# johnviljoen/f16_mpc_oop_py

Hardware: AMD Instinct MI355X
Metric: F16 env steps/sec (hifi Nguyen model, explicit Euler dt=1ms, batch 4096 per GPU) (higher is better)
Workload: dtype f64

## Files before the change

f16_mpc_oop_py_amd/csrc/f16_dynamics.hip:

```cpp
#include <hip/hip_runtime.h>
#include <stdlib.h>

#include <type_traits>

#include "../../include/f16_hip.h"
#include "f16_ctx.h"
#include "f16_plant.hpp"
#include "f16_rollout_common.hpp"
#include "f16_plant_quad.hpp"
#include "f16_mppi.hpp"
#include "f16_gain_sched.hpp"

namespace f16 {

struct CostArgs : SchedArgs {
  const double *x0;
  const double *x_ref;
  const double *u_ref;
  double *x_end;
  long B0, ld0;
  f16_cost_weights w;
};
struct GainSchedArgs : SchedArgs {
  f16_gain_grid grid;
// ... 533 lines not shown
#pragma unroll
        for (int k = 0; k < 3; ++k) { ls[k] = xt[k][lane]; ldm[k] = xt[3 + k][lane]; ts[k] = xt[6 + k][lane]; td[k] = xt[9 + k][lane]; }
        Totals tt;
        compose_totals(ls, ldm, ts, td, a.xcg, tt);
        if (wave == 0) {
          if (live) {
            p.qbar = xt[12][lane]; p.ps = xt[13][lane];
            st |= xst[0][lane] | xst[1][lane] | xst[2][lane] | xst[3][lane];
            plant_forces(xa, p, tt.Cx, tt.Cy, tt.Cz, xd);
#pragma unroll
            for (int k = 0; k < 9; ++k) x[k] += xd[k] * a.dt;
          }
        } else {
          if (live) {
            plant_moments(x[9], x[10], x[11], xt[12][lane], tt.Cl, tt.Cm, tt.Cn, xd);
#pragma unroll
            for (int k = 9; k < 12; ++k) x[k] += xd[k] * a.dt;
          }
          if (tr && --until_store == 0) {
            until_store = a.traj_every;
            if (valid) {
#pragma unroll
              for (int k = 9; k < 12; ++k) __builtin_nontemporal_store(x[k], tr + k * a.ld);
            }
            tr += 18 * a.ld;
          }
        }
      }
    }
#ifdef F16_EXP_STAMP4W
    if (lane == 0 && blockIdx.x == 0 && a.traj) {
      double *d = a.traj + 18 * a.ld * 2 + wave * 4;
      d[0] = (double)tD; d[1] = (double)tA; d[2] = (double)tB; d[3] = (double)tC;
    }
#endif
    if (valid && wave != 1) {
      bool finite = true;
      const int k0 = wave == 0 ? 0 : (wave == 2 ? 9 : 12), k1 = wave == 0 ? 9 : (wave == 2 ? 12 : 18);
#pragma unroll
      for (int k = 0; k < 18; ++k)
        if (k >= k0 && k < k1) { finite = finite && isfinite(x[k]); a.out[k * a.ld + b] = x[k]; }
      if (st & ST_ENVELOPE) st |= envelope_state_bits(x) & (((1 << k1) - (1 << k0)) << 8);
      if (a.status) atomicOr(&a.status[b], st | (finite ? 0 : ST_NONFINITE));
      if (LQR && wave == 3 && a.u_out) {
        a.u_out[b] = u[0];
#pragma unroll
        for (int i = 0; i < 3; ++i) a.u_out[(1 + i) * a.ld + b] = ul[i];
      }
    }
    __syncthreads();
  }
}

template <int GROUPS, bool LQR = false, bool SCHED = false>
__global__ __launch_bounds__(256 * GROUPS) void k_rollout_q(RolloutArgs<SCHED> a) {
  constexpr int NA = 16 * GROUPS;
  constexpr bool G1 = GROUPS == 1;
  __shared__ __attribute__((aligned(16))) double tab[TABLE_IMAGE_DOUBLES];
  __shared__ double xs[18][NA], xt[11][NA];
  __shared__ int xenv[3][NA], xst[2][NA];
  __shared__ double xpsi[G1 ? 4 : 3][NA];
#ifdef F16_EXP_STAMPQ
  const unsigned long long tstage0 = __builtin_amdgcn_s_memtime();
#endif
  {
    const double2 *src = reinterpret_cast<const double2 *>(a.tab);
    double2 *dst = reinterpret_cast<double2 *>(tab);
    for (int i = threadIdx.x; i < TABLE_IMAGE_DOUBLES / 2; i += 256 * GROUPS) dst[i] = src[i];
    __syncthreads();
  }
#ifdef F16_EXP_STAMPQ
  const unsigned long long tstage = __builtin_amdgcn_s_memtime() - tstage0;
#endif
  const int role = G1 ? __builtin_amdgcn_readfirstlane((threadIdx.x >> 6) & 3) : (threadIdx.x >> 6) & 3;
  const int grp = threadIdx.x >> 8, lane = threadIdx.x & 63, ac = 16 * grp + (lane >> 2), s = lane & 3;
  const bool envchk = !(a.flags & FLAG_NO_ENVELOPE);
  for (long b0 = (long)blockIdx.x * NA; b0 < a.B; b0 += (long)gridDim.x * NA) {
    const bool valid = b0 + ac < a.B;
    const long b = valid ? b0 + ac : a.B - 1;
    double x[18];
#pragma unroll
    for (int k = 0; k < 18; ++k) x[k] = a.out[k * a.ld + b];
    double ucmd = a.u[s * a.ld + b];
    double kr0 = 0, kr1 = 0, kr2 = 0, dm0 = 0, dm1 = 0, dm2 = 0, ulast = ucmd;
    if (LQR && role == 3) {
      const long row = 9 * (s > 0 ? s - 1 : 0) + 4;
      kr0 = a.K[row * a.ld + b]; kr1 = a.K[(row + 1) * a.ld + b]; kr2 = a.K[(row + 2) * a.ld + b];
      dm0 = a.dem[b]; dm1 = a.dem[a.ld + b]; dm2 = a.dem[2 * a.ld + b];
    }
    double xact = s == 0 ? x[12] : (s == 1 ? x[13] : (s == 2 ? x[14] : x[15]));
    int st = a.status ? a.status[b] : 0;
    double *tr = a.traj ? a.traj + b : nullptr;
    int until_store = a.traj_every;
    QuadCell qc = quad_cell_none();
    LongCorners klong = {};
    LatCorners klat = {};
    RowAhead<1, false> ra;
    double dmq = 0;
    const int rs = LQR && s == 3 ? 2 : s;
    if constexpr (SCHED) {
      dmq = s == 0 ? dm0 : (s == 1 ? dm1 : dm2);
      ra.init(a, LQR ? 3 : 4, a.out + b, rs * a.ld, role == 3);
      ra.settle();
    }
#ifdef F16_EXP_STAMPQ
    unsigned long long tA = 0, tB = 0, tC = 0, tD = 0, t0 = __builtin_amdgcn_s_memtime();
#if F16_EXP_STAMPQ + 0 == 2
#define QSTAMP_WAIT 0xC07F
#else
#define QSTAMP_WAIT 0
#endif
#define QSTAMP(acc) { __builtin_amdgcn_s_waitcnt(QSTAMP_WAIT); unsigned long long t1 = __builtin_amdgcn_s_memtime(); acc += t1 - t0; t0 = t1; }
#else
#define QSTAMP(acc)
#endif
    if constexpr (G1) {
      switch (role) {
        case 0: {
          constexpr int wave = 0;
#include "f16_quad_steps.inc"
        } break;
        case 1: {
          constexpr int wave = 1;
#include "f16_quad_steps.inc"
        } break;
        case 2: {
          constexpr int wave = 2;
#include "f16_quad_steps.inc"
        } break;
        default: {
          constexpr int wave = 3;
#include "f16_quad_steps.inc"
        } break;
      }
    } else {
      const int wave = role;
#include "f16_quad_steps.inc"
    }
#ifdef F16_EXP_STAMPQ
    if (lane == 0 && blockIdx.x == 0 && a.traj) {
      double *d = a.traj + 18 * a.ld * 2 + role * 4;
      d[0] = (double)tD; d[1] = (double)tA; d[2] = (double)tB; d[3] = (double)tC;
      a.traj[18 * a.ld * 2 + a.ld + role] = (double)tstage;
    }
#endif
    if (valid) {
      if (role == 2 && s == 0) {
        bool finite = true;
#pragma unroll
        for (int k = 0; k < 9; ++k) { finite = finite && isfinite(x[k]); a.out[k * a.ld + b] = x[k]; }
        if (st & ST_ENVELOPE) st |= envelope_state_bits(x) & (0x1FF << 8);
        if (a.status) atomicOr(&a.status[b], st | (finite ? 0 : ST_NONFINITE));
      } else if (role == 1 && s == 0) {
        bool finite = true;
#pragma unroll
        for (int k = 9; k < 12; ++k) { finite = finite && isfinite(x[k]); a.out[k * a.ld + b] = x[k]; }
        if (st & ST_ENVELOPE) st |= envelope_state_bits(x) & (0x7 << 17);
        if (a.status) atomicOr(&a.status[b], st | (finite ? 0 : ST_NONFINITE));
      } else if (role == 3) {
        a.out[(12 + s) * a.ld + b] = xact;
        bool finite = isfinite(xact);
        if (s < 2) { const double v = s == 0 ? x[16] : x[17]; finite = finite && isfinite(v); a.out[(16 + s) * a.ld + b] = v; }
        if (st & ST_ENVELOPE) {
          const double lim = s == 1 ? 25.0 : (s == 2 ? 21.5 : 30.0);
          if (s == 0 ? (xact < 1000 || xact > 19000) : (xact < -lim || xact > lim)) st |= 1 << (8 + 12 + s);
          if (s == 0 && (x[16] < 0. || x[16] > 25)) st |= 1 << (8 + 16);
        }
        if (a.status) atomicOr(&a.status[b], st | (finite ? 0 : ST_NONFINITE));
        if (LQR && a.u_out) a.u_out[s * a.ld + b] = ulast;
      }
    }
    __syncthreads();
  }
}

struct LinArgsL {
  double *x;
  const double *Ad, *Bd, *K, *xref, *u0;
  double *trx, *tru;
  long B, ld;
  int nsteps, every;
  unsigned track;
};
__global__ __launch_bounds__(64, 1) void k_rollout_lqr_linear(LinArgsL a) {
  const long b = (long)blockIdx.x * 64 + threadIdx.x;
  if (b >= a.B) return;
  double A[81], Bm[27], K[27], x[9], xr[9], u0[3];
#pragma unroll
  for (int e = 0; e < 81; ++e) A[e] = a.Ad[e * a.ld + b];
#pragma unroll
  for (int e = 0; e < 27; ++e) { Bm[e] = a.Bd[e * a.ld + b]; K[e] = a.K[e * a.ld + b]; }
#pragma unroll
  for (int j = 0; j < 9; ++j) { x[j] = a.x[j * a.ld + b]; xr[j] = a.xref[j * a.ld + b]; }
#pragma unroll
// ... 70 lines not shown
  if (int rc = check_common(ctx, x, xdot, B, ld)) return rc;
  if (!u) return set_error(F16_EINVAL, "u is NULL");
  if (B == 0) return F16_OK;
  DynArgs a = base_args<DynArgs>(ctx, B, ld, xcg, fi_flag, flags, status);
  a.x = x; a.u = u; a.out = xdot;
  const Geometry g = geometry(B, fi_flag);
  by_block(g, [&](auto block) {
    constexpr int BLOCK = decltype(block)::value;
    if (fi_flag == 0) hipLaunchKernelGGL((k_xdot<BLOCK, 0>), dim3(g.grid), dim3(BLOCK), 0, (hipStream_t)stream, a);
    else hipLaunchKernelGGL((k_xdot<BLOCK, -1>), dim3(g.grid), dim3(BLOCK), 0, (hipStream_t)stream, a);
  });
  return hip_check(hipGetLastError(), "f16_xdot_batch launch");
}

extern "C" int f16_nlplant_batch(f16_ctx *ctx, const double *xu, double *xdot, int32_t *status, long B, long ld,
                                 double xcg, int fi_flag, unsigned flags, void *stream) {
  if (int rc = check_common(ctx, xu, xdot, B, ld)) return rc;
  if (B == 0) return F16_OK;
  DynArgs a = base_args<DynArgs>(ctx, B, ld, xcg, fi_flag, flags, status);
  a.x = xu; a.out = xdot;
  if (B <= 256) {
    hipLaunchKernelGGL((k_nlplant<64, false>), dim3((unsigned)((B + 63) / 64)), dim3(64), 0, (hipStream_t)stream, a);
  } else {
    const Geometry g = geometry(B, fi_flag);
    by_block(g, [&](auto block) {
      constexpr int BLOCK = decltype(block)::value;
      hipLaunchKernelGGL((k_nlplant<BLOCK, true>), dim3(g.grid), dim3(BLOCK), 0, (hipStream_t)stream, a);
    });
  }
  return hip_check(hipGetLastError(), "f16_nlplant_batch launch");
}

#ifdef F16_RK4_512
constexpr bool RK4_512 = true;
#else
constexpr bool RK4_512 = false;
#endif
template <bool LQR, bool SCHED, bool COST, int STAGES = 1, bool GS = false>
static int rollout_dispatch(f16_ctx *ctx, RolloutArgsGS<SCHED, COST, GS> &a, void *stream) {
  const hipStream_t st = (hipStream_t)stream;
  const long B = a.B;
  const bool hifi = a.fi == 1;
  static const long max4w = [] { const char *e = getenv("F16_ROLLOUT_4W_MAXB"); return e ? atol(e) : 64L * 256; }();
  static const long maxq = [] { const char *e = getenv("F16_ROLLOUT_QUAD_MAXB"); return e ? atol(e) : 16L * 256; }();
  const char *const what = COST ? "f16_rollout_cost launch" : "f16_rollout launch";
  if (a.flags & F16_FLAG_ONE_LANE) {
    if constexpr (GS) hipLaunchKernelGGL((k_rollout_exact_gs<STAGES>), one_lane_grid(B), dim3(64), 0, st, a);
    else
    hipLaunchKernelGGL((k_rollout_exact<LQR, SCHED, COST, STAGES>), one_lane_grid(B), dim3(64), 0, st, a);
    return hip_check(hipGetLastError(), what);
  }
  if constexpr (!COST && STAGES == 1 && !GS) {
    if (hifi && B <= 2 * maxq) {
      if (B <= maxq) hipLaunchKernelGGL((k_rollout_q<1, LQR, SCHED>), dim3((unsigned)((B + 15) / 16)), dim3(256), 0, st, a);
      else hipLaunchKernelGGL((k_rollout_q<2, LQR, SCHED>), dim3((unsigned)((B + 31) / 32)), dim3(512), 0, st, a);
      return hip_check(hipGetLastError(), what);
    }
    if (hifi && B <= max4w) {
      hipLaunchKernelGGL((k_rollout_4w<LQR, SCHED>), dim3((unsigned)((B + 63) / 64)), dim3(256), 0, st, a);
      return hip_check(hipGetLastError(), what);
    }
  }
  constexpr bool WIDE = STAGES == 1 || RK4_512;
  Geometry g = geometry(B, a.fi, WIDE ? 512 : 256);
#ifdef F16_FAST_DIV
  static const int use_i32 = [] { const char *e = getenv("F16_ROLLOUT_I32"); return e ? atoi(e) : 1; }();
  if constexpr (WIDE) if (hifi && use_i32 && g.block == 512) {
    a.tab32 = ctx->d_tab32;
    if constexpr (GS) hipLaunchKernelGGL((k_rollout_i_gs<512, STAGES>), dim3(g.grid), dim3(512), 0, st, a);
    else
    hipLaunchKernelGGL((k_rollout_i<512, LQR, SCHED, COST, STAGES>), dim3(g.grid), dim3(512), 0, st, a);
    return hip_check(hipGetLastError(), what);
  }
#endif
  if (LQR && g.block == 512) g.block = 256;
  by_block(g, [&](auto block) {
    constexpr int BLOCK = decltype(block)::value;
    if constexpr (GS && BLOCK < 512) {
      if (a.fi == 0) hipLaunchKernelGGL((k_rollout_gs<BLOCK, 0, STAGES>), dim3(g.grid), dim3(BLOCK), 0, st, a);
      else hipLaunchKernelGGL((k_rollout_gs<BLOCK, -1, STAGES>), dim3(g.grid), dim3(BLOCK), 0, st, a);
    } else
    if constexpr (!((LQR || !WIDE) && BLOCK == 512)) {
      if (a.fi == 0) hipLaunchKernelGGL((k_rollout<BLOCK, 0, LQR, SCHED, COST, STAGES>), dim3(g.grid), dim3(BLOCK), 0, st, a);
      else hipLaunchKernelGGL((k_rollout<BLOCK, -1, LQR, SCHED, COST, STAGES>), dim3(g.grid), dim3(BLOCK), 0, st, a);
    }
  });
  return hip_check(hipGetLastError(), what);
}

struct PlantRollout {
  const char *missing;
  const double *x;
  const double *u;
  double *out;
  double *traj;
  int32_t *status;
  long B, ld;
  int nsteps, traj_every;
  double dt, xcg;
  int fi;
  unsigned flags;
  const double *seq = nullptr;
  int hold = 1;
  const double *K = nullptr, *dem = nullptr;
  double *u_out = nullptr;
  long B0 = 0, ld0 = 0;
  const double *x_ref = nullptr, *u_ref = nullptr;
// ... 217 lines not shown
```

f16_mpc_oop_py_amd/csrc/f16_plant.hpp:

```cpp
#pragma once
#include <hip/hip_runtime.h>

#include "f16_tables.h"

namespace f16 {

constexpr int ST_ALPHA1 = 1, ST_ALPHA2 = 2, ST_BETA = 4, ST_EL = 8, ST_ENVELOPE = 16, ST_NONFINITE = 32;
constexpr unsigned FLAG_FIX_CLR = 1u, FLAG_NO_ENVELOPE = 2u, FLAG_NO_CELL_CACHE = 16u;

#define F16_DEV __device__ __forceinline__

#ifdef F16_FAST_DIV
#define F16_DIVC(x, c) ((x) * (1.0 / (c)))
#else
#define F16_DIVC(x, c) ((x) / (c))
#endif

__device__ __forceinline__ double f16_rcp(double x) {
#ifdef F16_FAST_DIV
  double r = __builtin_amdgcn_rcp(x);
  r = fma(r, fma(-x, r, 1.0), r);
  r = fma(r, fma(-x, r, 1.0), r);
  return r;
#else
// ... 29 lines not shown
  static F16_DEV double kvv(double k, double b, double c) { return fma_svv(k, b, c); }
};
struct KVector {
  static F16_DEV double vvk(double a, double b, double k) { return fma_vvv(a, b, k); }
  static F16_DEV double kvv(double k, double b, double c) { return fma_vvv(k, b, c); }
};
F16_DEV void in_vgpr(double &x) { asm volatile("" : "+v"(x)); }
template <typename T>
F16_DEV void table_in_vgprs(T &t) {
  double *d = reinterpret_cast<double *>(&t);
#pragma unroll
  for (unsigned i = 0; i < sizeof(T) / sizeof(double); ++i) in_vgpr(d[i]);
}

struct PowK {
  double log2e, ln2_hi, ln2_lo, nln2_hi, nln2_lo, two_thirds;
  double E[10];
  double L[7];
};
constexpr PowK POW_K = {
    1.44269504088896338700e+00, 6.93147180559945286227e-01, 2.31904681384629955842e-17, -6.93147180559945286227e-01,
    -2.31904681384629955842e-17, 6.66666666666666629659e-01,
    {2.50223225676461415e-08, 2.76309034901126543e-07, 2.75575145458253105e-06, 2.48014910390950412e-05, 1.98412695891155217e-04,
     1.38888889459163820e-03, 8.33333333345504315e-03, 4.16666666665197541e-02, 1.66666666666664770e-01, 5.00000000000001221e-01},
    {1.53670161652585818e-01, 1.52503063567000663e-01, 1.81863527724766383e-01, 2.22221384831011309e-01, 2.85714293974435540e-01,
     3.99999999961319630e-01, 6.66666666666728247e-01}};

struct LogQuot {
  double h, l;
  int e;
};
template <typename OP = KScalar>
F16_DEV LogQuot log_k_quot(const PowK &K, double x) {
  const double m = __builtin_amdgcn_frexp_mant(x);
  const bool lo = m < K.two_thirds;
  const double sc = lo ? 2.0 : 1.0;
  const int e = __builtin_amdgcn_frexp_exp(x) + (lo ? -1 : 0);
  const double ym1 = fma(m, sc, -1.0), yp1 = fma(m, sc, 1.0);
  const double ylo = fma(m, sc, -(yp1 + -1.0));
  double r = __builtin_amdgcn_rcp(yp1);
  r = fma(fma(-yp1, r, 1.0), r, r);
  r = fma(fma(-yp1, r, 1.0), r, r);
  const double q = ym1 * r;
  const double p = yp1 * q;
  const double pl = fma(q, ylo, fma(q, yp1, -p));
  const double s25 = fma(yp1, q, pl);
  const double s27 = pl - fma(-yp1, q, s25);
  const double d28 = ym1 - s25;
  const double d32 = d28 + (((ym1 - d28) - s25) - s27);
  const double h = fma(r, d32, q);
  const double l = fma(r, d32, -fma(-ym1, r, h));
  return {h, l, e};
}
template <typename OP = KScalar>
F16_DEV double log_k_sum(const PowK &K, double x, const LogQuot &qt) {
  const double h = qt.h, l = qt.l;
  const int e = qt.e;
  const double z = h * h;
  double c = OP::vvk(z, K.L[0], K.L[1]);
#pragma unroll
  for (int k = 2; k < 7; ++k) c = OP::vvk(z, c, K.L[k]);
  const double a44 = __builtin_ldexp(h, 1), a45 = __builtin_ldexp(l, 1);
  const double t46 = h * z;
  const double u48 = fma(t46, c, a44);
  const double u50 = fma(t46, c, -(u48 - a44));
  const double u51 = a45 + u50;
  const double u52 = u48 + u51;
  const double u54 = u51 - (u52 - u48);
  const double f = (double)e;
  const double g56n = f * K.nln2_hi;
  const double g59 = OP::kvv(K.ln2_lo, f, OP::kvv(K.ln2_hi, f, g56n));
  const double g60 = OP::kvv(K.ln2_hi, f, g59);
  const double g62 = g59 - OP::kvv(K.nln2_hi, f, g60);
  const double w63 = g60 + u52;
  const double w64 = w63 - g60;
  const double w68 = (u52 - w64) + (g60 - (w63 - w64));
  const double v69 = g62 + u54;
  const double v70 = v69 - g62;
  const double v74 = (u54 - v70) + (g62 - (v69 - v70));
  const double k75 = v69 + w68;
  const double k76 = w63 + k75;
  const double k80 = k76 + (v74 + (k75 - (k76 - w63)));
  double res = __builtin_fabs(x) == __builtin_inf() ? x : k80;
  res = x < 0.0 ? __builtin_nan("") : res;
  return x == 0.0 ? -__builtin_inf() : res;
}
template <typename OP = KScalar>
F16_DEV double log_k(const PowK &K, double x) {
  return log_k_sum<OP>(K, x, log_k_quot<OP>(K, x));
}

template <typename OP = KScalar>
F16_DEV double exp_k(const PowK &K, double x) {
  const double n = rint(x * K.log2e);
  const double r = OP::kvv(K.nln2_lo, n, OP::kvv(K.nln2_hi, n, x));
  double c = OP::vvk(r, K.E[0], K.E[1]);
#pragma unroll
  for (int k = 2; k < 10; ++k) c = OP::vvk(r, c, K.E[k]);
  c = fma(r, c, 1.0);
  c = fma(r, c, 1.0);
  double res = __builtin_ldexp(c, (int)n);
  res = x > 1024.0 ? __builtin_inf() : res;
  return x < -1075.0 ? 0.0 : res;
}

struct AtmosAlt {
  double tfac, temp, t4;
};
F16_DEV AtmosAlt atmos_alt(double alt) {
  AtmosAlt h;
  h.tfac = 1 - .703e-5 * alt;
  h.temp = 519.0 * h.tfac;
  if (alt >= 35000.0) h.temp = 390;
#ifdef F16_FAST_POW
// ... 897 lines not shown
```

f16_mpc_oop_py_amd/csrc/f16_plant_quad.hpp:

```cpp
#pragma once
#include "f16_plant.hpp"

namespace f16 {

template <int J>
F16_DEV double quad_bcast(double v) {
  constexpr int ctrl = J | (J << 2) | (J << 4) | (J << 6);
  int lo = __double2loint(v), hi = __double2hiint(v);
  lo = __builtin_amdgcn_mov_dpp(lo, ctrl, 0xF, 0xF, true);
  hi = __builtin_amdgcn_mov_dpp(hi, ctrl, 0xF, 0xF, true);
  return __hiloint2double(hi, lo);
}

template <int J>
F16_DEV int quad_bcast_i(int v) {
  constexpr int ctrl = J | (J << 2) | (J << 4) | (J << 6);
  return __builtin_amdgcn_mov_dpp(v, ctrl, 0xF, 0xF, true);
}

F16_DEV void quad_taken_here_1(double &v) { asm volatile("" : "+v"(v)); }
F16_DEV void quad_taken_here_1(int &v) { asm volatile("" : "+v"(v)); }
template <typename... T>
F16_DEV void quad_taken_here(T &...v) { (quad_taken_here_1(v), ...); }

F16_DEV void quad_store_sample(const double (&smp)[5], double *tr, int s, long ld) {
#pragma unroll
  for (int j = 0; j < 5; ++j) {
    const int kk = s + 4 * j;
    if (kk < 18) __builtin_nontemporal_store(smp[j], tr + kk * ld);
  }
}

struct QuadBr { BrCell c; int ja, jb, jd; bool offa, offb, offd; };
template <bool USE_D2, typename TP>
F16_DEV BrRaw quad_br_load(TP T, double alpha, double beta, double el, int s, int &nX, double &vX) {
  const int ax = s < 2 ? s : 2;
  const int gel = USE_D2 ? (int)(el >= 0.0) : (el >= -10.0) + (el >= 0.0) + (el >= 10.0);
  const int offX = ax == 0 ? OFF_BP_A1 : (ax == 1 ? OFF_BP_B1 : (USE_D2 ? OFF_BP_D2 : OFF_BP_D1));
  nX = ax == 0 ? N_A1 : (ax == 1 ? N_B1 : (USE_D2 ? N_D2 : N_D1));
  vX = ax == 0 ? alpha : (ax == 1 ? beta : el);
  const int gX = ax == 0 ? alpha_guess(alpha) : (ax == 1 ? beta_guess(beta) : gel);
  return br_load(T + offX, nX, gX);
}
F16_DEV QuadBr quad_br_cells(const BrRaw &r, int nX, double vX) {
  QuadBr q;
  bool off;
  q.c = br_cell(r, nX, vX, off);
  q.ja = quad_bcast_i<0>(q.c.j); q.jb = quad_bcast_i<1>(q.c.j); q.jd = quad_bcast_i<2>(q.c.j);
  const int o = off ? 1 : 0;
  q.offa = quad_bcast_i<0>(o) != 0; q.offb = quad_bcast_i<1>(o) != 0; q.offd = quad_bcast_i<2>(o) != 0;
  return q;
}

struct QuadCell { int ja, jb, jd; double x0, x1; };
F16_DEV QuadCell quad_cell_none() { QuadCell c; c.ja = c.jb = c.jd = 0; c.x0 = c.x1 = __builtin_nan(""); return c; }
template <bool USE_D2, bool CACHE, typename TP>
F16_DEV QuadBr quad_br_cached(TP T, double alpha, double beta, double el, int s, unsigned flags, QuadCell &cc, bool &hit) {
  const double v = s == 0 ? alpha : (s == 1 ? beta : el);
  const bool in = cc.x0 <= v && v < cc.x1;
  QuadBr q;
  hit = CACHE && !(flags & FLAG_NO_CELL_CACHE) && __builtin_amdgcn_ballot_w64(!in) == 0;
  if (hit) {
    q.c.j = 0; q.c.v = v; q.c.x0 = cc.x0; q.c.x1 = cc.x1;
    q.ja = cc.ja; q.jb = cc.jb; q.jd = cc.jd;
    q.offa = q.offb = q.offd = false;
  } else {
    int nX; double vX;
    const BrRaw rx = quad_br_load<USE_D2>(T, alpha, beta, el, s, nX, vX);
    F16_PHASE();
    q = quad_br_cells(rx, nX, vX);
    if (CACHE) { cc.ja = q.ja; cc.jb = q.jb; cc.jd = q.jd; cc.x0 = q.c.x0; cc.x1 = q.c.x1; }
  }
  return q;
}
F16_DEV void quad_br_axes(const QuadBr &q, Axis &a, Axis &b, Axis &d) {
  const Axis own = br_axis(q.c);
  a.j = q.ja; a.l = quad_bcast<0>(own.l); a.m = quad_bcast<0>(own.m);
  b.j = q.jb; b.l = quad_bcast<1>(own.l); b.m = quad_bcast<1>(own.m);
  d.j = q.jd; d.l = quad_bcast<2>(own.l); d.m = quad_bcast<2>(own.m);
}

struct LongCorners {
  Q4 qlo, qhi, q0, qlef;
  double g0, g1, m0, m1, h0, h1, e0, e1, r0, r1, p0, p1, b0, b1, hr0, hr1, hp0, hp1, a45;
};
struct LatCorners {
  Q4 qlo, qhi, q0, qy, qr, qa, ql, qal;
  double a45;
};

template <bool PIN>
F16_DEV double lerp_d(double f1, double f2, const Axis &a) {
  if constexpr (PIN) return __builtin_fma(a.l, f2, a.m * f1);
  else return lerp(f1, f2, a);
}

struct QuadIn {
  double alpha, beta, el, dail, drud, dlef, P, Q, R, kq, kb;
};
F16_DEV QuadIn quad_inputs(const double *xu) {
  const double B = 30.0, cbar = 11.32, r2d = 180.0 / 3.141592653589793;
  QuadIn in;
  double vt = xu[6];
  if (vt <= 0.01) vt = 0.01;
  in.alpha = xu[7] * r2d; in.beta = xu[8] * r2d;
  in.P = xu[9]; in.Q = xu[10]; in.R = xu[11];
  in.el = xu[13];
  in.dail = F16_DIVC(xu[14], 21.5);
  in.drud = F16_DIVC(xu[15], 30.0);
  in.dlef = 1 - F16_DIVC(xu[16], 25.0);
#ifdef F16_FAST_DIV
  const double r2vt = f16_rcp(2 * vt);
  in.kq = cbar * r2vt; in.kb = B * r2vt;
#else
  in.kq = cbar / (2 * vt); in.kb = B / (2 * vt);
#endif
  return in;
}

#ifdef F16_EXP_STAMPQ2
__device__ unsigned long long g_qstamp[8];
#define Q2STAMP(i) { __builtin_amdgcn_s_waitcnt(0); const unsigned long long t1_ = __builtin_amdgcn_s_memtime(); if (blockIdx.x == 0 && (threadIdx.x & 63) == 0) g_qstamp[i] += t1_ - tq_; tq_ = t1_; }
#else
#define Q2STAMP(i)
#endif
template <bool CACHE, typename TP>
F16_DEV double quad_long(TP T, const double *xu, int s, double xcg, unsigned flags, QuadCell &cc, LongCorners &kept, double &latd,
                         int &status) {
#ifdef F16_EXP_STAMPQ2
  unsigned long long tq_ = __builtin_amdgcn_s_memtime();
#endif
  const QuadIn in = quad_inputs(xu);
  Q2STAMP(0)
  const int k = s < 2 ? s : 2;
  bool hit;
  const QuadBr qb = quad_br_cached<false, CACHE>(T, in.alpha, in.beta, in.el, s, flags, cc, hit);
  Q2STAMP(1)
  LongCorners fresh;
  LongCorners &c = CACHE ? kept : fresh;
  const bool hi_a = qb.ja > N_A2 - 2;
  if (!CACHE || !hit) {
    c.a45 = T[OFF_BP_A1 + N_A2 - 1];
    const int j2 = hi_a ? N_A2 - 2 : qb.ja;
    const int n1 = qb.jb * N_A1 + qb.ja, n2 = qb.jb * N_A2 + j2;
    struct { int j; } ca = {qb.ja}, cd = {qb.jd};
    constexpr int SA = S_G3A, SB = S_G3A * N_A1, SD = S_G3A * N_A1 * N_B1;
    TP p = T + OFF_G3A + n1 * SA + k;
    c.qlo = ld4(p + cd.j * SD, SA, SB); c.qhi = ld4(p + (cd.j + 1) * SD, SA, SB); c.q0 = ld4(p + D1_ZERO_NODE * SD, SA, SB);
    c.qlef = ld4(T + OFF_G2B + n2 * S_G2B + k, S_G2B, S_G2B * N_A2);
    TP g = T + OFF_G1A + ca.j * S_G1A, h = T + OFF_G1B + j2 * S_G1B;
    c.g0 = g[3 * k]; c.g1 = g[S_G1A + 3 * k]; c.m0 = g[11]; c.m1 = g[S_G1A + 11];
    c.h0 = h[3 * k]; c.h1 = h[S_G1B + 3 * k];
    c.e0 = T[OFF_ETA + cd.j]; c.e1 = T[OFF_ETA + cd.j + 1];
    const int ir = k == 0 ? 1 : (k == 1 ? 7 : 4), ib = k == 1 ? 9 : 10;
    c.r0 = g[ir]; c.r1 = g[S_G1A + ir]; c.p0 = g[ir + 1]; c.p1 = g[S_G1A + ir + 1]; c.b0 = g[ib]; c.b1 = g[S_G1A + ib];
    c.hr0 = h[ir]; c.hr1 = h[S_G1B + ir]; c.hp0 = h[ir + 1]; c.hp1 = h[S_G1B + ir + 1];
  }
  if (qb.offa) status |= ST_ALPHA1 | ST_ALPHA2;
  if (qb.offb) status |= ST_BETA;
  if (qb.offd) status |= ST_EL;
  if (hi_a && in.alpha > c.a45) status |= ST_ALPHA2;
  Q2STAMP(2)
  F16_PHASE();
  Axis a1, b, d1;
  quad_br_axes(qb, a1, b, d1);
  Axis a2 = a1;
  if (hi_a) { a2.j = N_A2 - 2; a2.l = 1.0; a2.m = 0.0; }
  const W4 W1 = bil_weights(a1, b), W2 = bil_weights(a2, b);
  const double Cf = lerp_d<CACHE>(bil4w(c.qlo, a1, b, W1), bil4w(c.qhi, a1, b, W1), d1);
  const double C0 = bil4w(c.q0, a1, b, W1);
  const double dC = bil4w(c.qlef, a2, b, W2) - C0;
  const double Cq = lerp(c.g0, c.g1, a1), dCm = lerp(c.m0, c.m1, a1), dq = lerp(c.h0, c.h1, a2), eta = lerp(c.e0, c.e1, d1);
  const double dql = k == 1 ? dC : dq;
  double tot = Cf * (k == 2 ? eta : 1.0) + dC * in.dlef + in.kq * (Cq + dql * in.dlef) * in.Q + (k == 2 ? dCm : 0.0);
  const double Cz_tot = quad_bcast<1>(tot);
  if (k == 2) tot += Cz_tot * (0.35 - xcg);
  double Cr = lerp(c.r0, c.r1, a1);
  if (k == 2 && !(flags & FLAG_FIX_CLR)) Cr = 0.0;
  const double Cp = lerp(c.p0, c.p1, a1), Cb = lerp(c.b0, c.b1, a1);
  const double dCr = lerp(c.hr0, c.hr1, a2), dCp = lerp(c.hp0, c.hp1, a2);
  latd = in.kb * (Cr + dCr * in.dlef) * in.R + in.kb * (Cp + dCp * in.dlef) * in.P + (k == 0 ? 0.0 : Cb * in.beta);
  Q2STAMP(3)
  return tot;
}

template <bool CACHE, typename TP>
F16_DEV double quad_lat(TP T, const double *xu, int s, unsigned flags, QuadCell &cc, LatCorners &kept, int &status) {
  const QuadIn in = quad_inputs(xu);
  const int k = s < 2 ? s : 2;
  bool hit;
  const QuadBr qb = quad_br_cached<true, CACHE>(T, in.alpha, in.beta, in.el, s, flags, cc, hit);
  LatCorners fresh;
  LatCorners &c = CACHE ? kept : fresh;
  const bool hi_a = qb.ja > N_A2 - 2;
  if (!CACHE || !hit) {
    c.a45 = T[OFF_BP_A1 + N_A2 - 1];
    const int j2 = hi_a ? N_A2 - 2 : qb.ja;
    const int n1 = qb.jb * N_A1 + qb.ja, n2 = qb.jb * N_A2 + j2;
    struct { int j; } cd = {qb.jd};
    constexpr int SA3 = S_G3B, SB3 = S_G3B * N_A1, SD3 = S_G3B * N_A1 * N_B1;
    TP p3 = T + OFF_G3B + n1 * SA3 + (k > 0 ? k - 1 : 0);
    c.qlo = ld4(p3 + cd.j * SD3, SA3, SB3); c.qhi = ld4(p3 + (cd.j + 1) * SD3, SA3, SB3); c.q0 = ld4(p3 + D2_ZERO_NODE * SD3, SA3, SB3);
    constexpr int SA2 = S_G2A, SB2 = S_G2A * N_A1;
    TP pa = T + OFF_G2A + n1 * SA2;
    c.qy = ld4(pa, SA2, SB2); c.qr = ld4(pa + 1 + k, SA2, SB2); c.qa = ld4(pa + 4 + k, SA2, SB2);
    constexpr int SAB = S_G2B, SBB = S_G2B * N_A2;
    TP pb = T + OFF_G2B + n2 * SAB;
    c.ql = ld4(pb + 3 + k, SAB, SBB); c.qal = ld4(pb + 6 + k, SAB, SBB);
  }
  if (qb.offa) status |= ST_ALPHA1 | ST_ALPHA2;
  if (qb.offb) status |= ST_BETA;
  if (qb.offd) status |= ST_EL;
  if (hi_a && in.alpha > c.a45) status |= ST_ALPHA2;
  F16_PHASE();
  Axis a1, b, d2;
  quad_br_axes(qb, a1, b, d2);
  Axis a2 = a1;
  if (hi_a) { a2.j = N_A2 - 2; a2.l = 1.0; a2.m = 0.0; }
  const W4 W1 = bil_weights(a1, b), W2 = bil_weights(a2, b);
  const double C3 = lerp_d<CACHE>(bil4w(c.qlo, a1, b, W1), bil4w(c.qhi, a1, b, W1), d2), C30 = bil4w(c.q0, a1, b, W1);
  const double Cy = bil4w(c.qy, a1, b, W1), Cr30 = bil4w(c.qr, a1, b, W1), Ca20 = bil4w(c.qa, a1, b, W1);
  const double Clef = bil4w(c.ql, a2, b, W2), Ca20lef = bil4w(c.qal, a2, b, W2);
  const double base = k == 0 ? Cy : C3, base0 = k == 0 ? Cy : C30;
  const double dlefC = Clef - base0;
  const double dr30 = Cr30 - base0;
  const double da20 = Ca20 - base0, da20lef = Ca20lef - Clef - da20;
  return base + dlefC * in.dlef + (da20 + da20lef * in.dlef) * in.dail + dr30 * in.drud;
}

}
```

f16_mpc_oop_py_amd/csrc/f16_quad_steps.inc:

```
    [[maybe_unused]] SinCosK ksc = {};
    [[maybe_unused]] PowK kpw = {};
    [[maybe_unused]] bool env_h = false;
    [[maybe_unused]] AtmosAlt ah = {};
    [[maybe_unused]] LogQuot lq = {};
    if constexpr (G1) {
      if (wave == 0 || wave == 2) ksc = reloaded(QUAD_K.sc);
      if (wave == 3) kpw = reloaded(QUAD_K.pw);
      if (wave == 2) table_in_vgprs(ksc);
      if (wave == 0) { in_vgpr(ksc.S[7]); in_vgpr(ksc.C[8]); }
      if (wave == 3) { in_vgpr(kpw.E[0]); in_vgpr(kpw.L[0]); }
      if (wave == 0 && s == 0) {
        double sp, cp;
        F16_SINCOS_K(ksc, x[5], &sp, &cp);
        xpsi[1][ac] = sp; xpsi[2][ac] = cp;
      }
      if (wave == 2) {
        env_h = envchk && (x[2] < 0 || x[2] > 100000);
        if (s == 0) {
#pragma unroll
          for (int k = 0; k < 6; ++k) xs[k][ac] = x[k];
        }
      }
      if (wave == 3) {
        ah = atmos_alt(x[2]);
        lq = log_k_quot(kpw, ah.tfac);
        quad_taken_here(ah.tfac, ah.temp, ah.t4, lq.h, lq.l, lq.e);
      }
      if (wave != 3) {
#pragma unroll
        for (int k = 0; k < 18; ++k)
          if (!(wave == 2 ? k < 9 : (wave == 1 && k >= 9 && k < 12))) x[k] = 0;
      }
    }
    for (int t = 0; t <= a.nsteps; ++t) {
      if (wave == 2) {
        if constexpr (G1) {
          xenv[0][ac] = env_h | (envchk & ((x[6] < 0) | (x[6] > 900) | (x[7] < -20.) | (x[7] > 90) | (x[8] < -30.) | (x[8] > 30)));
          xs[6 + (s < 3 ? s : 2)][ac] = s == 0 ? x[6] : (s == 1 ? x[7] : x[8]);
        } else {
          xenv[0][ac] = envchk && (x[2] < 0 || x[2] > 100000 || x[6] < 0 || x[6] > 900 || x[7] < -20. || x[7] > 90 ||
                                   x[8] < -30. || x[8] > 30);
          if (s == 0) {
#pragma unroll
            for (int k = 0; k < 9; ++k) xs[k][ac] = x[k];
          }
        }
      } else if (wave == 1) {
        xenv[1][ac] = envchk && (x[9] < -300 || x[9] > 300 || x[10] < -100 || x[10] > 100 || x[11] < -50 || x[11] > 50);
        if (s < 3) xs[9 + s][ac] = s == 0 ? x[9] : (s == 1 ? x[10] : x[11]);
      } else if (wave == 3) {
        const double lim = s == 1 ? 25.0 : (s == 2 ? 21.5 : 30.0);
        const bool bad = s == 0 ? (xact < 1000 || xact > 19000) : (xact < -lim || xact > lim);
        const bool badl = x[16] < 0. || x[16] > 25;
        if (s == 0) xenv[2][ac] = 0;
        xs[12 + s][ac] = xact;
        if (s < 2) xs[16 + s][ac] = s == 0 ? x[16] : x[17];
        __builtin_amdgcn_wave_barrier();
        if (envchk && (bad || badl)) xenv[2][ac] = 1;
      }
      QSTAMP(tD)
      __syncthreads();
      QSTAMP(tA)
      double xa[17];
      int env_any = 0;
      if constexpr (G1) {
        env_any = xenv[0][ac] | xenv[1][ac] | xenv[2][ac];
#pragma unroll
        for (int k = 0; k < 17; ++k) xa[k] = xs[k][ac];
        if (wave == 2) { xa[3] = x[3]; xa[4] = x[4]; xa[6] = x[6]; xa[7] = x[7]; xa[8] = x[8]; }
        if (wave == 1) { xa[9] = x[9]; xa[10] = x[10]; xa[11] = x[11]; }
      }
      [[maybe_unused]] double smp[5] = {0, 0, 0, 0, 0};
      [[maybe_unused]] bool sample_due = false;
      if constexpr (G1) {
        if (wave == 2) {
#pragma unroll
          for (int j = 0; j < 5; ++j) smp[j] = xs[s + 4 * j < 18 ? s + 4 * j : s][ac];
          asm volatile("" ::: "memory");
        }
      }
      if (wave == 2 && tr && t > 0 && --until_store == 0) {
        until_store = a.traj_every;
        if constexpr (G1) {
          sample_due = true;
        } else {
          if (valid) {
#pragma unroll
            for (int j = 0; j < 5; ++j) {
              const int kk = s + 4 * j;
              if (kk < 18) __builtin_nontemporal_store(xs[kk][ac], tr + kk * a.ld);
            }
          }
          tr += 18 * a.ld;
        }
      }
      if (t == a.nsteps) {
        if constexpr (G1) {
          if (sample_due && valid) quad_store_sample(smp, tr, s, a.ld);
        }
        break;
      }
      if constexpr (!G1) {
        env_any = xenv[0][ac] | xenv[1][ac] | xenv[2][ac];
#pragma unroll
        for (int k = 0; k < 17; ++k) xa[k] = xs[k][ac];
      }
      if ((!G1 || wave != 0) && env_any) st |= ST_ENVELOPE;
      const bool live = !(st & ST_ENVELOPE);
      double xd[9] = {0, 0, 0, 0, 0, 0, 0, 0, 0};
      double U = 0, V = 0, W = 0, s_t = 0, c_t = 0, s_phi = 0, c_phi = 0, cb = 0, vtc = 0, r1 = 0, r2 = 0, r3 = 0;
      double fu0 = 0, fv0 = 0, fw0 = 0, mo0 = 0, mo1 = 0, mo2 = 0;
      bool newrow = false;
      if constexpr (SCHED) newrow = ra.due(a, LQR ? 3 : 4);
      if (wave == 0) {
        int sa_ = 0;
        double latd;
        const double tot = quad_long<G1>((const double *)tab, xa, s, a.xcg, a.flags, qc, klong, latd, sa_);
        if (s < 3) { xt[s][ac] = tot; xt[8 + s][ac] = latd; }
        xst[0][ac] = sa_;
      } else if (wave == 1) {
        int sa_ = 0;
        const double tot = quad_lat<G1>((const double *)tab, xa, s, a.flags, qc, klat, sa_);
        if (s < 3) xt[3 + s][ac] = tot;
        xst[1][ac] = sa_;
        {
          const double Jy = 55814.0, Jxz = 982.0, Jz = 63100.0, Jx = 9496.0;
          const double rden = 1.0 / (9496.0 * 63100.0 - 982.0 * 982.0);
          const double P = x[9], Q = x[10], R = x[11];
          mo0 = (Jxz * (Jx - Jy + Jz) * P * Q - (Jz * (Jz - Jy) + Jxz * Jxz) * Q * R) * rden;
          mo1 = F16_DIVC((Jz - Jx) * P * R - Jxz * (P * P - R * R), Jy);
          mo2 = ((Jx * (Jx - Jy) + Jxz * Jxz) * P * Q - Jxz * (Jx - Jy + Jz) * Q * R) * rden;
        }
        if constexpr (G1) quad_taken_here(mo0, mo1, mo2);
      } else if (wave == 2) {
        double ang;
        if constexpr (G1) {
          ang = xa[7];
          ang = s == 2 ? xa[8] : ang;
          ang = s == 1 ? xa[4] : ang;
          ang = s == 0 ? xa[3] : ang;
        } else
          ang = s == 0 ? xa[3] : (s == 1 ? xa[4] : (s == 2 ? xa[5] : xa[7]));
        double sn, cs, sb, s_psi, c_psi;
        if constexpr (G1) F16_SINCOS_KC(KVector, ksc, ang, &sn, &cs);
        else F16_SINCOS(ang, &sn, &cs);
        if constexpr (G1) {
          if (sample_due) {
            if (valid) quad_store_sample(smp, tr, s, a.ld);
            tr += 18 * a.ld;
          }
        }
        if constexpr (G1) { sb = quad_bcast<2>(sn); cb = quad_bcast<2>(cs); } else F16_SINCOS(xa[8], &sb, &cb);
        s_phi = quad_bcast<0>(sn); c_phi = quad_bcast<0>(cs);
        s_t = quad_bcast<1>(sn); c_t = quad_bcast<1>(cs);
        if constexpr (G1) { s_psi = xpsi[1][ac]; c_psi = xpsi[2][ac]; } else { s_psi = quad_bcast<2>(sn); c_psi = quad_bcast<2>(cs); }
        const double sal = quad_bcast<3>(sn), cal = quad_bcast<3>(cs);
        vtc = xa[6];
        if (vtc <= 0.01) vtc = 0.01;
        U = vtc * cal * cb; V = vtc * sb; W = vtc * sal * cb;
        const double P = xa[9], Q = xa[10], R = xa[11];
#ifdef F16_FAST_DIV
        const double rct = f16_rcp(c_t);
        const double tt = s_t * rct;
#elif defined(F16_FAST_TAN)
        const double rct = 0.0, tt = s_t / c_t;
#else
        const double rct = 0.0, tt = tan(xa[4]);
#endif
        xd[0] = U * (c_t * c_psi) + V * (s_phi * c_psi * s_t - c_phi * s_psi) + W * (c_phi * s_t * c_psi + s_phi * s_psi);
        xd[1] = U * (c_t * s_psi) + V * (s_phi * s_psi * s_t + c_phi * c_psi) + W * (c_phi * s_t * s_psi - s_phi * c_psi);
        xd[2] = U * s_t - V * (s_phi * c_t) - W * (c_phi * c_t);
        xd[3] = P + tt * (Q * s_phi + R * c_phi);
        xd[4] = Q * c_phi - R * s_phi;
#ifdef F16_FAST_DIV
        xd[5] = (Q * s_phi + R * c_phi) * rct;
        r1 = f16_rcp(vtc); r2 = f16_rcp(U * U + W * W); r3 = f16_rcp(vtc * vtc * cb);
#else
        xd[5] = (Q * s_phi + R * c_phi) / c_t;
        (void)rct;
#endif
        {
          const double g = 32.17, m = 636.94;
          fu0 = R * V - Q * W - g * s_t + F16_DIVC(xa[12], m);
          fv0 = P * W - R * U + g * c_t * s_phi;
          fw0 = Q * U - P * V + g * c_t * c_phi;
          if (live) {
#pragma unroll
            for (int k = 0; k < 6; ++k) x[k] += xd[k] * a.dt;
          }
          if constexpr (G1) if (s == 0) { xpsi[0][ac] = x[5]; xpsi[3][ac] = x[2]; }
        }
        if constexpr (G1) quad_taken_here(U, V, W, vtc, r1, r2, r3, fu0, fv0, fw0);
      } else {
        double vt = xa[6];
        if (vt <= 0.01) vt = 0.01;
        double mach, qbar, ps;
        double pw = 0;
        if constexpr (G1) {
          quad_taken_here(ah.tfac, lq.h, lq.l, lq.e);
          pw = exp_k(kpw, 0.14 * log_k_sum(kpw, ah.tfac, lq));
          atmos_air(ah, vt, mach, qbar, ps, [pw](double) { return pw; });
        } else
          atmos_dev(xa[2], vt, mach, qbar, ps);
        if (s == 0) { xt[6][ac] = qbar; xt[7][ac] = ps; }
        if (live) {
          const double lim = s == 1 ? 25.0 : (s == 2 ? 21.5 : 30.0), rate = s == 1 ? 60.0 : (s == 2 ? 80.0 : 120.0);
          double uc = ucmd;
          if (LQR) {
            if constexpr (SCHED) { dm0 = quad_bcast<0>(dmq); dm1 = quad_bcast<1>(dmq); dm2 = quad_bcast<2>(dmq); }
            const double ua = lqr_action(kr0, kr1, kr2, dm0 - xa[9], dm1 - xa[10], dm2 - xa[11], ucmd);
            uc = s > 0 ? ua : ucmd;
            ulast = uc;
          }
          const double dth = actuator_rate(ucmd, 1000, 19000, 1.0, xact, 10000);
          const double dsf = actuator_rate(uc, -lim, lim, 20.2, xact, rate);
          double lf1_dot, lf2_dot;
          if constexpr (G1)
            upd_lef_with(0.0, xa[6], xa[7], x[17], x[16], qbar, ps, lf1_dot, lf2_dot,
                         [pw, &ah](double, double V_, double &m_, double &q_, double &p_) {
                           atmos_air(ah, V_, m_, q_, p_, [pw](double) { return pw; });
                         });
          else
            upd_lef_dev(xa[2], xa[6], xa[7], x[17], x[16], qbar, ps, lf1_dot, lf2_dot);
          xact += (s == 0 ? dth : dsf) * a.dt;
          x[16] += lf2_dot * a.dt;
          x[17] += lf1_dot * a.dt;
        }
        if constexpr (SCHED) if (newrow) {
          int rv;
          asm volatile("v_mbcnt_lo_u32_b32 %0, -1, 0\n\tv_mbcnt_hi_u32_b32 %0, -1, %0" : "=v"(rv));
          rv &= 3;
          if (LQR && rv == 3) rv = 2;
          ra.take(a, LQR ? 3 : 4, LQR ? &dmq : &ucmd, a.out + b, rv * a.ld);
          if (LQR) ulast = ucmd;
        }
      }
      QSTAMP(tB)
      __syncthreads();
      QSTAMP(tC)
      if (wave == 2) {
        int sx = 0;
        double t0_ = 0, t1_ = 0, t3_ = 0, t8_ = 0, t6_ = 0;
        if constexpr (G1) {
          sx = xst[0][ac] | xst[1][ac];
          t0_ = xt[0][ac]; t1_ = xt[1][ac]; t3_ = xt[3][ac]; t8_ = xt[8][ac]; t6_ = xt[6][ac];
          __builtin_amdgcn_sched_barrier(0);
          env_h = envchk & ((x[2] < 0) | (x[2] > 100000));
          if (s == 0) {
#pragma unroll
            for (int k = 0; k < 6; ++k) xs[k][ac] = x[k];
          }
        }
        if (live) {
          if constexpr (!G1) { sx = xst[0][ac] | xst[1][ac]; t0_ = xt[0][ac]; t1_ = xt[1][ac]; t3_ = xt[3][ac]; t8_ = xt[8][ac]; t6_ = xt[6][ac]; }
          st |= sx;
          const double Cx = t0_, Cz = t1_, Cy = t3_ + t8_, qbar = t6_;
          const double m = 636.94, S = 300.0;
          const double qsm = F16_DIVC(qbar * S, m);
          const double Udot = fu0 + qsm * Cx;
          const double Vdot = fv0 + qsm * Cy;
          const double Wdot = fw0 + qsm * Cz;
#ifdef F16_FAST_DIV
          xd[6] = (U * Udot + V * Vdot + W * Wdot) * r1;
          xd[7] = (U * Wdot - W * Udot) * r2;
          xd[8] = (Vdot * vtc - V * xd[6]) * r3;
#else
          xd[6] = (U * Udot + V * Vdot + W * Wdot) / vtc;
          xd[7] = (U * Wdot - W * Udot) / (U * U + W * W);
          xd[8] = (Vdot * vtc - V * xd[6]) / (vtc * vtc * cb);
#endif
#pragma unroll
          for (int k = 6; k < 9; ++k) x[k] += xd[k] * a.dt;
        }
      } else if (wave == 1) {
        if (live) {
          const double Cy = xt[3][ac] + xt[8][ac];
          const double Cn = xt[4][ac] + xt[9][ac] - Cy * (0.35 - a.xcg) * (11.32 / 30.0);
          const double Cl = xt[5][ac] + xt[10][ac];
          const double Jy = 55814.0, Jxz = 982.0, Jz = 63100.0, Jx = 9496.0, S = 300.0;
          const double rden = 1.0 / (9496.0 * 63100.0 - 982.0 * 982.0);
          const double qs = xt[6][ac] * S;
          const double L_tot = Cl * qs * 30.0, M_tot = xt[2][ac] * qs * 11.32, N_tot = Cn * qs * 30.0;
          x[9] += (mo0 + (Jz * L_tot + Jxz * N_tot) * rden) * a.dt;
          x[10] += (mo1 + F16_DIVC(M_tot, Jy)) * a.dt;
          x[11] += (mo2 + (Jx * N_tot + Jxz * L_tot) * rden) * a.dt;
        }
      } else if constexpr (G1) {
        if (wave == 0 && s == 0) {
          double sp, cp;
          F16_SINCOS_K(ksc, xpsi[0][ac], &sp, &cp);
          xpsi[1][ac] = sp; xpsi[2][ac] = cp;
        } else if (wave == 3) {
          ah = atmos_alt(xpsi[3][ac]);
          lq = log_k_quot(kpw, ah.tfac);
          quad_taken_here(ah.tfac, ah.temp, ah.t4, lq.h, lq.l, lq.e);
        }
      }
    }
```

Before: 4.880 billion.

## Add fifth wave for trajectory sampling and precompute log poly and cell reciprocals

Measured after the change: 5.217 billion (median of 6 runs). 6.9% higher.

```diff
diff --git a/f16_mpc_oop_py_amd/csrc/f16_dynamics.hip b/f16_mpc_oop_py_amd/csrc/f16_dynamics.hip
--- a/f16_mpc_oop_py_amd/csrc/f16_dynamics.hip
+++ b/f16_mpc_oop_py_amd/csrc/f16_dynamics.hip
@@ -609,10 +609,12 @@
   }
 }
 
+constexpr int quad_block_threads(int groups) { return groups == 1 ? 320 : 256 * groups; }
 template <int GROUPS, bool LQR = false, bool SCHED = false>
-__global__ __launch_bounds__(256 * GROUPS) void k_rollout_q(RolloutArgs<SCHED> a) {
+__global__ __launch_bounds__(quad_block_threads(GROUPS)) void k_rollout_q(RolloutArgs<SCHED> a) {
   constexpr int NA = 16 * GROUPS;
   constexpr bool G1 = GROUPS == 1;
+  constexpr int NT = quad_block_threads(GROUPS);
   __shared__ __attribute__((aligned(16))) double tab[TABLE_IMAGE_DOUBLES];
   __shared__ double xs[18][NA], xt[11][NA];
   __shared__ int xenv[3][NA], xst[2][NA];
@@ -623,14 +625,14 @@
   {
     const double2 *src = reinterpret_cast<const double2 *>(a.tab);
     double2 *dst = reinterpret_cast<double2 *>(tab);
-    for (int i = threadIdx.x; i < TABLE_IMAGE_DOUBLES / 2; i += 256 * GROUPS) dst[i] = src[i];
+    for (int i = threadIdx.x; i < TABLE_IMAGE_DOUBLES / 2; i += NT) dst[i] = src[i];
     __syncthreads();
   }
 #ifdef F16_EXP_STAMPQ
   const unsigned long long tstage = __builtin_amdgcn_s_memtime() - tstage0;
 #endif
-  const int role = G1 ? __builtin_amdgcn_readfirstlane((threadIdx.x >> 6) & 3) : (threadIdx.x >> 6) & 3;
-  const int grp = threadIdx.x >> 8, lane = threadIdx.x & 63, ac = 16 * grp + (lane >> 2), s = lane & 3;
+  const int role = G1 ? __builtin_amdgcn_readfirstlane(threadIdx.x >> 6) : (threadIdx.x >> 6) & 3;
+  const int grp = G1 ? 0 : threadIdx.x >> 8, lane = threadIdx.x & 63, ac = 16 * grp + (lane >> 2), s = lane & 3;
   const bool envchk = !(a.flags & FLAG_NO_ENVELOPE);
   for (long b0 = (long)blockIdx.x * NA; b0 < a.B; b0 += (long)gridDim.x * NA) {
     const bool valid = b0 + ac < a.B;
@@ -685,6 +687,10 @@
           constexpr int wave = 2;
 #include "f16_quad_steps.inc"
         } break;
+        case 4: {
+          constexpr int wave = 4;
+#include "f16_quad_steps.inc"
+        } break;
         default: {
           constexpr int wave = 3;
 #include "f16_quad_steps.inc"
@@ -696,7 +702,7 @@
     }
 #ifdef F16_EXP_STAMPQ
     if (lane == 0 && blockIdx.x == 0 && a.traj) {
-      double *d = a.traj + 18 * a.ld * 2 + role * 4;
+      double *d = a.traj + 18 * a.ld * 2 + (role < 4 ? role * 4 : 2 * a.ld);
       d[0] = (double)tD; d[1] = (double)tA; d[2] = (double)tB; d[3] = (double)tC;
       a.traj[18 * a.ld * 2 + a.ld + role] = (double)tstage;
     }
@@ -873,7 +879,7 @@
   }
   if constexpr (!COST && STAGES == 1 && !GS) {
     if (hifi && B <= 2 * maxq) {
-      if (B <= maxq) hipLaunchKernelGGL((k_rollout_q<1, LQR, SCHED>), dim3((unsigned)((B + 15) / 16)), dim3(256), 0, st, a);
+      if (B <= maxq) hipLaunchKernelGGL((k_rollout_q<1, LQR, SCHED>), dim3((unsigned)((B + 15) / 16)), dim3(quad_block_threads(1)), 0, st, a);
       else hipLaunchKernelGGL((k_rollout_q<2, LQR, SCHED>), dim3((unsigned)((B + 31) / 32)), dim3(512), 0, st, a);
       return hip_check(hipGetLastError(), what);
     }
diff --git a/f16_mpc_oop_py_amd/csrc/f16_plant.hpp b/f16_mpc_oop_py_amd/csrc/f16_plant.hpp
--- a/f16_mpc_oop_py_amd/csrc/f16_plant.hpp
+++ b/f16_mpc_oop_py_amd/csrc/f16_plant.hpp
@@ -105,14 +105,28 @@
   const double l = fma(r, d32, -fma(-ym1, r, h));
   return {h, l, e};
 }
+struct LogPoly {
+  double z, c;
+};
+template <typename OP = KScalar>
+F16_DEV LogPoly log_k_poly(const PowK &K, const LogQuot &qt) {
+  const double z = qt.h * qt.h;
+  double c = OP::vvk(z, K.L[0], K.L[1]);
+#pragma unroll
+  for (int k = 2; k < 7; ++k) c = OP::vvk(z, c, K.L[k]);
+  return {z, c};
+}
+template <typename OP = KScalar>
+F16_DEV double log_k_tail(const PowK &K, double x, const LogQuot &qt, const LogPoly &pl);
 template <typename OP = KScalar>
 F16_DEV double log_k_sum(const PowK &K, double x, const LogQuot &qt) {
+  return log_k_tail<OP>(K, x, qt, log_k_poly<OP>(K, qt));
+}
+template <typename OP>
+F16_DEV double log_k_tail(const PowK &K, double x, const LogQuot &qt, const LogPoly &pl) {
   const double h = qt.h, l = qt.l;
   const int e = qt.e;
-  const double z = h * h;
-  double c = OP::vvk(z, K.L[0], K.L[1]);
-#pragma unroll
-  for (int k = 2; k < 7; ++k) c = OP::vvk(z, c, K.L[k]);
+  const double z = pl.z, c = pl.c;
   const double a44 = __builtin_ldexp(h, 1), a45 = __builtin_ldexp(l, 1);
   const double t46 = h * z;
   const double u48 = fma(t46, c, a44);
diff --git a/f16_mpc_oop_py_amd/csrc/f16_plant_quad.hpp b/f16_mpc_oop_py_amd/csrc/f16_plant_quad.hpp
--- a/f16_mpc_oop_py_amd/csrc/f16_plant_quad.hpp
+++ b/f16_mpc_oop_py_amd/csrc/f16_plant_quad.hpp
@@ -31,7 +31,7 @@
   }
 }
 
-struct QuadBr { BrCell c; int ja, jb, jd; bool offa, offb, offd; };
+struct QuadBr { BrCell c; int ja, jb, jd; bool offa, offb, offd; double l; };
 template <bool USE_D2, typename TP>
 F16_DEV BrRaw quad_br_load(TP T, double alpha, double beta, double el, int s, int &nX, double &vX) {
   const int ax = s < 2 ? s : 2;
@@ -44,6 +44,7 @@
 }
 F16_DEV QuadBr quad_br_cells(const BrRaw &r, int nX, double vX) {
   QuadBr q;
+  q.l = 0;
   bool off;
   q.c = br_cell(r, nX, vX, off);
   q.ja = quad_bcast_i<0>(q.c.j); q.jb = quad_bcast_i<1>(q.c.j); q.jd = quad_bcast_i<2>(q.c.j);
@@ -52,29 +53,54 @@
   return q;
 }
 
-struct QuadCell { int ja, jb, jd; double x0, x1; };
-F16_DEV QuadCell quad_cell_none() { QuadCell c; c.ja = c.jb = c.jd = 0; c.x0 = c.x1 = __builtin_nan(""); return c; }
+struct QuadCell { int ja, jb, jd; double x0, x1, rw; };
+F16_DEV QuadCell quad_cell_none() { QuadCell c; c.ja = c.jb = c.jd = 0; c.x0 = c.x1 = __builtin_nan(""); c.rw = 0; return c; }
 template <bool USE_D2, bool CACHE, typename TP>
 F16_DEV QuadBr quad_br_cached(TP T, double alpha, double beta, double el, int s, unsigned flags, QuadCell &cc, bool &hit) {
   const double v = s == 0 ? alpha : (s == 1 ? beta : el);
-  const bool in = cc.x0 <= v && v < cc.x1;
   QuadBr q;
-  hit = CACHE && !(flags & FLAG_NO_CELL_CACHE) && __builtin_amdgcn_ballot_w64(!in) == 0;
+  q.l = 0;
+  if constexpr (CACHE) {
+    const unsigned long long keep = (flags & FLAG_NO_CELL_CACHE) ? 0ull : ~0ull;
+    const auto inside = __builtin_amdgcn_ballot_w64(cc.x0 <= v) & __builtin_amdgcn_ballot_w64(v < cc.x1) & keep;
+    hit = inside == __builtin_amdgcn_ballot_w64(true);
+  } else
+    hit = false;
   if (hit) {
     q.c.j = 0; q.c.v = v; q.c.x0 = cc.x0; q.c.x1 = cc.x1;
     q.ja = cc.ja; q.jb = cc.jb; q.jd = cc.jd;
     q.offa = q.offb = q.offd = false;
+#ifdef F16_FAST_DIV
+    q.l = (v - cc.x0) * cc.rw;
+#endif
   } else {
     int nX; double vX;
     const BrRaw rx = quad_br_load<USE_D2>(T, alpha, beta, el, s, nX, vX);
     F16_PHASE();
     q = quad_br_cells(rx, nX, vX);
-    if (CACHE) { cc.ja = q.ja; cc.jb = q.jb; cc.jd = q.jd; cc.x0 = q.c.x0; cc.x1 = q.c.x1; }
+    if (CACHE) {
+      cc.ja = q.ja; cc.jb = q.jb; cc.jd = q.jd; cc.x0 = q.c.x0; cc.x1 = q.c.x1;
+#ifdef F16_FAST_DIV
+      cc.rw = f16_rcp(q.c.x1 - q.c.x0);
+      q.l = q.c.v == q.c.x1 ? 1.0 : (q.c.v - q.c.x0) * cc.rw;
+#endif
+    }
   }
   return q;
 }
+template <bool CACHE>
 F16_DEV void quad_br_axes(const QuadBr &q, Axis &a, Axis &b, Axis &d) {
-  const Axis own = br_axis(q.c);
+  Axis own;
+#ifdef F16_FAST_DIV
+  if constexpr (CACHE) {
+    own.j = q.c.j; own.l = q.l;
+    quad_taken_here(own.l);
+    own.m = 1 - own.l;
+  } else
+    own = br_axis(q.c);
+#else
+  own = br_axis(q.c);
+#endif
   a.j = q.ja; a.l = quad_bcast<0>(own.l); a.m = quad_bcast<0>(own.m);
   b.j = q.jb; b.l = quad_bcast<1>(own.l); b.m = quad_bcast<1>(own.m);
   d.j = q.jd; d.l = quad_bcast<2>(own.l); d.m = quad_bcast<2>(own.m);
@@ -155,15 +181,15 @@
     const int ir = k == 0 ? 1 : (k == 1 ? 7 : 4), ib = k == 1 ? 9 : 10;
     c.r0 = g[ir]; c.r1 = g[S_G1A + ir]; c.p0 = g[ir + 1]; c.p1 = g[S_G1A + ir + 1]; c.b0 = g[ib]; c.b1 = g[S_G1A + ib];
     c.hr0 = h[ir]; c.hr1 = h[S_G1B + ir]; c.hp0 = h[ir + 1]; c.hp1 = h[S_G1B + ir + 1];
-  }
-  if (qb.offa) status |= ST_ALPHA1 | ST_ALPHA2;
-  if (qb.offb) status |= ST_BETA;
-  if (qb.offd) status |= ST_EL;
+    if (qb.offa) status |= ST_ALPHA1 | ST_ALPHA2;
+    if (qb.offb) status |= ST_BETA;
+    if (qb.offd) status |= ST_EL;
+  }
   if (hi_a && in.alpha > c.a45) status |= ST_ALPHA2;
   Q2STAMP(2)
   F16_PHASE();
   Axis a1, b, d1;
-  quad_br_axes(qb, a1, b, d1);
+  quad_br_axes<CACHE>(qb, a1, b, d1);
   Axis a2 = a1;
   if (hi_a) { a2.j = N_A2 - 2; a2.l = 1.0; a2.m = 0.0; }
   const W4 W1 = bil_weights(a1, b), W2 = bil_weights(a2, b);
@@ -207,14 +233,14 @@
     constexpr int SAB = S_G2B, SBB = S_G2B * N_A2;
     TP pb = T + OFF_G2B + n2 * SAB;
     c.ql = ld4(pb + 3 + k, SAB, SBB); c.qal = ld4(pb + 6 + k, SAB, SBB);
-  }
-  if (qb.offa) status |= ST_ALPHA1 | ST_ALPHA2;
-  if (qb.offb) status |= ST_BETA;
-  if (qb.offd) status |= ST_EL;
+    if (qb.offa) status |= ST_ALPHA1 | ST_ALPHA2;
+    if (qb.offb) status |= ST_BETA;
+    if (qb.offd) status |= ST_EL;
+  }
   if (hi_a && in.alpha > c.a45) status |= ST_ALPHA2;
   F16_PHASE();
   Axis a1, b, d2;
-  quad_br_axes(qb, a1, b, d2);
+  quad_br_axes<CACHE>(qb, a1, b, d2);
   Axis a2 = a1;
   if (hi_a) { a2.j = N_A2 - 2; a2.l = 1.0; a2.m = 0.0; }
   const W4 W1 = bil_weights(a1, b), W2 = bil_weights(a2, b);
diff --git a/f16_mpc_oop_py_amd/csrc/f16_quad_steps.inc b/f16_mpc_oop_py_amd/csrc/f16_quad_steps.inc
--- a/f16_mpc_oop_py_amd/csrc/f16_quad_steps.inc
+++ b/f16_mpc_oop_py_amd/csrc/f16_quad_steps.inc
@@ -3,6 +3,7 @@
     [[maybe_unused]] bool env_h = false;
     [[maybe_unused]] AtmosAlt ah = {};
     [[maybe_unused]] LogQuot lq = {};
+    [[maybe_unused]] LogPoly lp = {};
     if constexpr (G1) {
       if (wave == 0 || wave == 2) ksc = reloaded(QUAD_K.sc);
       if (wave == 3) kpw = reloaded(QUAD_K.pw);
@@ -24,7 +25,8 @@
       if (wave == 3) {
         ah = atmos_alt(x[2]);
         lq = log_k_quot(kpw, ah.tfac);
-        quad_taken_here(ah.tfac, ah.temp, ah.t4, lq.h, lq.l, lq.e);
+        lp = log_k_poly(kpw, lq);
+        quad_taken_here(ah.tfac, ah.temp, ah.t4, lq.h, lq.l, lq.e, lp.z, lp.c);
       }
       if (wave != 3) {
 #pragma unroll
@@ -73,13 +75,13 @@
       [[maybe_unused]] double smp[5] = {0, 0, 0, 0, 0};
       [[maybe_unused]] bool sample_due = false;
       if constexpr (G1) {
-        if (wave == 2) {
+        if (wave == 4) {
 #pragma unroll
           for (int j = 0; j < 5; ++j) smp[j] = xs[s + 4 * j < 18 ? s + 4 * j : s][ac];
           asm volatile("" ::: "memory");
         }
       }
-      if (wave == 2 && tr && t > 0 && --until_store == 0) {
+      if (wave == (G1 ? 4 : 2) && tr && t > 0 && --until_store == 0) {
         until_store = a.traj_every;
         if constexpr (G1) {
           sample_due = true;
@@ -105,7 +107,7 @@
 #pragma unroll
         for (int k = 0; k < 17; ++k) xa[k] = xs[k][ac];
       }
-      if ((!G1 || wave != 0) && env_any) st |= ST_ENVELOPE;
+      if ((!G1 || (wave != 0 && wave != 4)) && env_any) st |= ST_ENVELOPE;
       const bool live = !(st & ST_ENVELOPE);
       double xd[9] = {0, 0, 0, 0, 0, 0, 0, 0, 0};
       double U = 0, V = 0, W = 0, s_t = 0, c_t = 0, s_phi = 0, c_phi = 0, cb = 0, vtc = 0, r1 = 0, r2 = 0, r3 = 0;
@@ -144,12 +146,6 @@
         double sn, cs, sb, s_psi, c_psi;
         if constexpr (G1) F16_SINCOS_KC(KVector, ksc, ang, &sn, &cs);
         else F16_SINCOS(ang, &sn, &cs);
-        if constexpr (G1) {
-          if (sample_due) {
-            if (valid) quad_store_sample(smp, tr, s, a.ld);
-            tr += 18 * a.ld;
-          }
-        }
         if constexpr (G1) { sb = quad_bcast<2>(sn); cb = quad_bcast<2>(cs); } else F16_SINCOS(xa[8], &sb, &cb);
         s_phi = quad_bcast<0>(sn); c_phi = quad_bcast<0>(cs);
         s_t = quad_bcast<1>(sn); c_t = quad_bcast<1>(cs);
@@ -191,14 +187,19 @@
           if constexpr (G1) if (s == 0) { xpsi[0][ac] = x[5]; xpsi[3][ac] = x[2]; }
         }
         if constexpr (G1) quad_taken_here(U, V, W, vtc, r1, r2, r3, fu0, fv0, fw0);
+      } else if (G1 && wave == 4) {
+        if (sample_due) {
+          if (valid) quad_store_sample(smp, tr, s, a.ld);
+          tr += 18 * a.ld;
+        }
       } else {
         double vt = xa[6];
         if (vt <= 0.01) vt = 0.01;
         double mach, qbar, ps;
         double pw = 0;
         if constexpr (G1) {
-          quad_taken_here(ah.tfac, lq.h, lq.l, lq.e);
-          pw = exp_k(kpw, 0.14 * log_k_sum(kpw, ah.tfac, lq));
+          quad_taken_here(ah.tfac, lq.h, lq.l, lq.e, lp.z, lp.c);
+          pw = exp_k(kpw, 0.14 * log_k_tail(kpw, ah.tfac, lq, lp));
           atmos_air(ah, vt, mach, qbar, ps, [pw](double) { return pw; });
         } else
           atmos_dev(xa[2], vt, mach, qbar, ps);
@@ -293,7 +294,8 @@
         } else if (wave == 3) {
           ah = atmos_alt(xpsi[3][ac]);
           lq = log_k_quot(kpw, ah.tfac);
-          quad_taken_here(ah.tfac, ah.temp, ah.t4, lq.h, lq.l, lq.e);
+          lp = log_k_poly(kpw, lq);
+          quad_taken_here(ah.tfac, ah.temp, ah.t4, lq.h, lq.l, lq.e, lp.z, lp.c);
         }
       }
     }
```
